# google/qhbm-library

Measured on AMD Instinct MI355X. Metric: circuit-expectation evals/sec (samples×Pauli terms) at n qubits; VQT step time, higher is better.
Workload: dtype f32; 1 GPU; BASELINE configs[2] (20-qubit XXZ, depth 16, 4096-sample VQT step): 20-qubit XXZ(delta=0.5) open chain, HEA depth 16 (944 params), 4096 states in total = 4096 on rank 0 of 1, VQT step = values + adjoint VJP; n_qubits=20, layers=16, states_total=4096, states_per_gpu=4096, pauli_terms=57, observables=1, hamiltonian=xxz, mode=vqt, parallelism=batch-sharded x1, backend_world_size=1, forward_passes=7, adjoint_passes=9

## Files before the change

### qhbm-library_amd/csrc/engine.cpp

```cpp
#include <hip/hip_runtime.h>

#include <algorithm>
#include <cmath>
#include <cstdio>
#include <iterator>
#include <cstdlib>
#include <cstring>
#include <memory>
#include <optional>
#include <string>
#include <vector>

#include "../../include/qhbm_engine.h"
#include "kernels.h"
#include "plan_args.h"
#include "program.h"
#include "schedule.h"

using namespace qhbm;

namespace {

std::string g_create_error;

// ... 46 lines not shown
  std::vector<std::pair<std::vector<char>, std::unique_ptr<DevicePlan>>> adj_cache;
  int64_t fwd_plans_built = 0, adj_plans_built = 0;
  DevBuf<DevTerm> global_terms;
  DevBuf<int> param_slot_begin, param_slots;
  DevBuf<float> slot_factor;
  DevBuf<ShiftPhase> shift_phases;
  int n_shift_phases = 0;
  bool shift_ready = false;
  size_t coef_batch_programs = 0;
};

struct TimedEvent {
  hipEvent_t a, b;
  int kind;
};

}

struct qhbm_engine {
  int device = -1;
  std::string err;
  Model model;
  bool have_circuit = false;
  int opt_tile = 0, opt_adj_tile = 0, opt_profile = 0, opt_round = 0;
  int opt_full_fwd = 60, opt_full_adj = 60, opt_force_general = 0;
  int opt_meas_tile = 0;
  int opt_values_from_obs = 1;
  bool retained_mu = false;
  int opt_cph_wave_bits = 1;
  int opt_fwd_values_obs = -1;
  int opt_adj_stop_early = -1;
  int opt_adj_plan_search = 1;
  int opt_wide_last = -1;
  int opt_fwd_pair = 1;
  int opt_shift_prefix = 1;
  int opt_adj_relabel = 1;
  int opt_obs_xcd_states = -1;
  int opt_x_two_shear = 1;
  int opt_adj_exchange = 1;
  int retained_U = 0;
  bool retained_table = false;
  int state_grad_U = 0;
  int64_t opt_chunk = 0;
  int64_t opt_budget_mb = 0;
  size_t resolved_budget = 0;
  bool plans_valid = false;
  bool adj_valid = false;
  std::vector<std::pair<std::vector<char>, std::unique_ptr<DevicePlan>>> adj_cache;
  int64_t fwd_plans_built = 0, adj_plans_built = 0;
  bool model_uploaded = false;
  DevicePlan fwd, adj;
  DevBuf<DevTerm> terms, global_terms;
  DevBuf<ObsGroup> obs_groups;
  bool terms_by_op = false;
  DevBuf<ObsBTerm> obs_bterms;
  DevBuf<ObsBGroup> obs_bgroups;
  uint32_t n_obs_bgroups = 0;
  int opt_obs_block_bits = kObsBlockBits;
  int opt_obs_split_rows = 0;
  int opt_obs_kernel = -1;
  mutable int block_choice = -1;
  int opt_gather_multi = 0;
  int opt_multi_values = -1;
  DevBuf<uint64_t> probe_out;
  DevBuf<float> probe_sink;
  DevBuf<float> value_part;
// ... 234 lines not shown
  }
  for (size_t i = 0; i < args->size(); ++i) {
    PassArgs& a = (*args)[i];
    if ((a.flags & PASS_INIT_BASIS) && (a.flags & PASS_NO_ZERO_FILL))
      for (uint32_t k = 0; k < a.n_nonlocal; ++k) a.zero_mask |= 1u << a.nonlocal_pos[k];
    a.n_free = a.n_nonlocal - uint32_t(__builtin_popcount(a.zero_mask));
  }
}

namespace {

double pass_flops_per_amplitude(const Plan& plan, const Pass& p, const uint32_t* dyn = nullptr);

double adjoint_plan_seconds(const Plan& plan, const Model& m) {
  std::vector<PassArgs> args;
  std::vector<uint32_t> prog, tables;
  fill_args(plan, m, &args, &prog, &tables);
  const double amps = double(size_t(1) << plan.n_eff);
  double t = 0.0;
  for (size_t i = 0; i < args.size(); ++i) {
    const Pass& p = plan.passes[i];
    const double live = 1.0 / double(1ull << __builtin_popcount(args[i].zero_mask));
    int low_missing = 0;
    for (uint32_t k = 0; k < args[i].n_nonlocal; ++k) low_missing += args[i].nonlocal_pos[k] < 4;
    const double lines = std::min(1.0, live * double(1u << low_missing));
    const double write_share = (p.flags & PASS_RELABEL) ? 1.0 / double(1u << __builtin_popcount(p.frozen_new_local)) : 1.0;
    const double bytes = lines * amps * 8.0 * 2.0 * (1.0 + ((p.flags & PASS_STORE) ? write_share : 0.0));
    const double flops = live * amps * pass_flops_per_amplitude(plan, p);
    t += std::max(flops / 67e12, bytes / 5.5e12) + 0.1 * bytes / 5.5e12;
  }
  return t;
}

int build_plans(qhbm_engine* h) {
  if (h->plans_valid && h->adj_valid) return 0;
  if (!h->have_circuit) return fail(h, "qhbm_set_circuit has not been called");
  if (h->model.n_ops > kMaxOps) return fail(h, "too many observables (max 1024)");
  std::string err;
  if (!h->plans_valid) {
    h->adj_cache.clear();
    if (!build_plan(h->model, h->opt_tile, h->opt_round, false, &h->fwd.plan, &err, h->opt_full_fwd, h->opt_meas_tile,
                    h->opt_cph_wave_bits != 0, false, h->opt_wide_last))
      return fail(h, "forward plan: " + err);
    h->fwd.uploaded = false;
    ++h->fwd_plans_built;
  }
  const bool relabel = h->opt_adj_relabel != 0 && h->opt_adj_exchange != 0;
  auto plan_adjoint_of = [&](const Model& model, int tile, Plan* out, double* seconds, std::string* e) {
    if (!build_plan(model, tile, 0, true, out, e, h->opt_full_adj, 0, h->opt_cph_wave_bits != 0, relabel)) return false;
    *seconds = adjoint_plan_seconds(*out, model);
    if (!h->opt_adj_plan_search) return true;
    const std::vector<std::vector<uint32_t>> orders = out->candidate_orders;
    for (const std::vector<uint32_t>& order : orders) {
      Plan alt;
      std::string e2;
      if (!build_plan(model, tile, 0, true, &alt, &e2, h->opt_full_adj, 0, h->opt_cph_wave_bits != 0, relabel, -1, &order))
        continue;
      const double f = adjoint_plan_seconds(alt, model);
      if (std::getenv("QHBM_PLAN_DEBUG"))
        std::fprintf(stderr, "[plan] tile %d candidate with %zu passes: %.4g ms per state (kept so far: %zu passes, %.4g ms)\n", tile,
                     alt.passes.size(), f * 1e3, out->passes.size(), *seconds * 1e3);
      if (f < 0.99 * *seconds) { *out = std::move(alt); *seconds = f; }
    }
    return true;
  };
  auto plan_adjoint = [&](int tile, Plan* out, double* seconds, std::string* e) {
    bool any_live = false;
    for (const Gate& G : h->model.gates) any_live |= G.param_idx >= 0 && !h->model.frozen(G.param_idx);
    if (h->opt_adj_stop_early == 0 && !h->model.param_frozen.empty() && any_live) {
      Model whole = h->model;
      whole.stop_at_first_live_gate = false;
      return plan_adjoint_of(whole, tile, out, seconds, e);
    }
    if (!plan_adjoint_of(h->model, tile, out, seconds, e)) return false;
    if (h->opt_adj_stop_early < 0 && !h->model.param_frozen.empty() && out->dense_tail) {
      Model whole = h->model;
// ... 958 lines not shown
    for (int j = term_offsets[k]; j < term_offsets[k + 1]; ++j) bound += std::fabs(double(coeffs[j]));
    int e = 0;
    if (bound > 0.0) (void)std::frexp(bound, &e);
    e = std::max(-60, std::min(60, e));
    h->h_op_scale[size_t(k)] = float(std::ldexp(1.0, kValueFracBits - e));
    h->h_op_inv_scale[size_t(k)] = float(std::ldexp(1.0, e - kValueFracBits));
  }
  h->model.n_ops = n_ops;
  h->model.terms = std::move(terms);
  invalidate_plans(h);
  h->block_choice = -1;
  h->terms.release();
  return 0;
}

int qhbm_set_option(qhbm_engine* h, const char* name, int64_t value) {
  if (!h || !name) return 1;
  const std::string k(name);
  if (k == "tile_qubits") { h->opt_tile = int(value); invalidate_plans(h); h->block_choice = -1; }
  else if (k == "round_qubits") { h->opt_round = int(value); invalidate_plans(h); }
  else if (k == "force_general_kernels") h->opt_force_general = int(value);
  else if (k == "full_diag_threshold") { h->opt_full_fwd = int(value); invalidate_plans(h); }
  else if (k == "adjoint_full_diag_threshold") { h->opt_full_adj = int(value); invalidate_plans(h); }
  else if (k == "adjoint_tile_qubits") { h->opt_adj_tile = int(value); invalidate_plans(h); }
  else if (k == "adjoint_exchange") { h->opt_adj_exchange = int(value); invalidate_plans(h); }
  else if (k == "x_two_shear") { h->opt_x_two_shear = value != 0; invalidate_plans(h); h->adj_cache.clear(); h->dense.adj_cache.clear(); }
  else if (k == "adjoint_relabel") { h->opt_adj_relabel = int(value); invalidate_plans(h); }
  else if (k == "forward_pairs") h->opt_fwd_pair = int(value);
  else if (k == "shift_prefix_sharing") { h->opt_shift_prefix = int(value); h->shift_ready = false; }
  else if (k == "forward_values_from_observable") h->opt_fwd_values_obs = int(value);
  else if (k == "adjoint_stop_early") { h->opt_adj_stop_early = int(value); invalidate_plans(h); }
  else if (k == "adjoint_plan_search") { h->opt_adj_plan_search = int(value); invalidate_plans(h); }
  else if (k == "wide_last_pass") { h->opt_wide_last = int(value); invalidate_plans(h); }
  else if (k == "observable_xcd_states") h->opt_obs_xcd_states = int(value);
  else if (k == "observable_kernel") { h->opt_obs_kernel = int(value); h->block_choice = -1; }
  else if (k == "observable_split_rows") h->opt_obs_split_rows = value != 0;
  else if (k == "observable_block_bits") {
    if (value != kObsBlockBits && value != kObsBlockBitsSmall) return fail(h, "observable_block_bits: 12 or 13");
    h->opt_obs_block_bits = int(value); h->block_choice = -1; h->terms.release(); h->model_uploaded = false;
  }
  else if (k == "multi_observable_values") h->opt_multi_values = int(value);
  else if (k == "gather_multi_values") h->opt_gather_multi = int(value);
  else if (k == "observable_far_windows") { h->opt_far_windows = int(value); h->terms.release(); h->model_uploaded = false; }
  else if (k == "measure_tile_qubits") { h->opt_meas_tile = int(value); invalidate_plans(h); }
  else if (k == "values_from_observable") h->opt_values_from_obs = int(value);
  else if (k == "cph_wave_bits") { h->opt_cph_wave_bits = int(value); invalidate_plans(h); }
  else if (k == "chunk_states") h->opt_chunk = value;
  else if (k == "evolve_step_argument") {
    if (value < 1 || value > 64) return fail(h, "evolve_step_argument: 1 .. 64");
    h->opt_evolve_step = int(value);
  }
  else if (k == "workspace_budget_mb") h->opt_budget_mb = std::max<int64_t>(0, value);
  else if (k == "profile_events") h->opt_profile = int(value);
  else return fail(h, "unknown option '" + k + "'");
  return 0;
}

int qhbm_workspace_bytes(qhbm_engine* h, int U, int with_vjp, size_t* out) {
  if (!h || !out) return 1;
  if (int rc = build_plans(h)) return rc;
  const uint32_t cs = with_vjp ? adjoint_chunk_states(h, U) : chunk_states(h, U);
  size_t b = size_t(cs) * state_bytes(h) * (with_vjp ? 2 : 1);
  if (with_vjp) {
    b += size_t(U) * h->adj.plan.slot_gate.size() * sizeof(float);
    size_t rows = 0;
    for (const Pass& p : h->adj.plan.passes)
// ... 1020 lines not shown
    HIPCHK(h->vals_tmp.reserve(nv));
    d_out_vals = h->vals_tmp.p;
  }
  std::vector<float> up(nv);
  for (int k = 0; k < T; ++k) {
    for (size_t i = 0; i < nv; ++i) up[i] = (int(i % size_t(T)) == k) ? 1.f : 0.f;
    HIPCHK(hipMemcpyAsync(h->upstream_tmp.p, up.data(), nv * sizeof(float), hipMemcpyHostToDevice, s));
    HIPCHK(hipStreamSynchronize(s));
    if (int rc = adjoint_sweep(h, d_bits, U, d_params, h->upstream_tmp.p, d_out_vals, s)) return rc;
    HIPCHK(launch_scatter_jac(h->state_grad.p, uint32_t(U), uint32_t(h->adj.plan.slot_gate.size()),
                              h->param_slot_begin.p, h->param_slots.p, h->slot_factor.p, d_jac, uint32_t(T),
                              uint32_t(k), uint32_t(P), s));
  }
  return 0;
}

int qhbm_num_passes(qhbm_engine* h, int* forward_passes, int* backward_passes) {
  if (!h) return 1;
  if (int rc = build_plans(h)) return rc;
  if (forward_passes) *forward_passes = int(h->fwd.plan.passes.size());
  if (backward_passes) *backward_passes = int(h->adj.plan.passes.size());
  return 0;
}

int qhbm_describe_schedule(qhbm_engine* h, char* buf, size_t buf_len) {
  if (!h || !buf || !buf_len) return 1;
  if (int rc = build_plans(h)) return rc;
  std::string s = describe_plan(h->fwd.plan) + describe_plan(h->adj.plan);
  {
    char line[96];
    std::snprintf(line, sizeof(line), "adjoint time model: %.2f us per state\n", 1e6 * adjoint_plan_seconds(h->adj.plan, h->model));
    s += line;
  }
  if (!h->model.terms.empty()) {
    s += std::string("observable kernel: lambda = ") + (block_kernel(h) ? "observable_blocks_kernel" : "apply_observable_kernel");
    s += std::string(" values = ") + (gather_multi_mode(h) ? "apply_observable_kernel (an accumulator per observable)"
                                      : multi_value_mode(h) || (value_mode(h) && block_kernel(h)) ? "observable_blocks_kernel"
                                      : value_mode(h)                                            ? "apply_observable_kernel"
                                                                                                  : "measured in the passes");
    s += "\n";
  }
  std::snprintf(buf, buf_len, "%s", s.c_str());
  return 0;
}

int qhbm_kernel_time_ms(qhbm_engine* h, int reset, double* fwd_ms, int64_t* fwd_launches, double* bwd_ms,
                        int64_t* bwd_launches, double* obs_ms, int64_t* obs_launches) {
  if (!h) return 1;
  double ms[3] = {0.0, 0.0, 0.0};
  int64_t cnt[3] = {0, 0, 0};
  if (h->device >= 0 && !h->events.empty()) {
    HIPCHK(hipSetDevice(h->device));
    HIPCHK(hipEventSynchronize(h->events.back().b));
    for (auto& ev : h->events) {
      float t = 0.f;
      if (hipEventElapsedTime(&t, ev.a, ev.b) == hipSuccess) { ms[ev.kind] += t; ++cnt[ev.kind]; }
    }
  }
  if (fwd_ms) *fwd_ms = ms[0];
  if (fwd_launches) *fwd_launches = cnt[0];
  if (bwd_ms) *bwd_ms = ms[1];
  if (bwd_launches) *bwd_launches = cnt[1];
  if (obs_ms) *obs_ms = ms[2];
  if (obs_launches) *obs_launches = cnt[2];
  if (reset) {
    h->free_events.insert(h->free_events.end(), h->events.begin(), h->events.end());
// ... 236 lines not shown
  if (with_vjp) {
    std::vector<PassArgs> args;
    std::vector<uint32_t> prog, tables;
    fill_args(h->adj.plan, h->model, &args, &prog, &tables);
    for (size_t i = 0; i < args.size(); ++i) {
      const double live = 1.0 / double(1ull << __builtin_popcount(args[i].zero_mask));
      b += live * amps * pass_flops_per_amplitude(h->adj.plan, h->adj.plan.passes[i], dyn_b.empty() ? nullptr : dyn_b.data());
    }
  }
  if (fwd_flops) *fwd_flops = f;
  if (obs_flops) *obs_flops = o;
  if (bwd_flops) *bwd_flops = b;
  return 0;
}

extern "C" {

int qhbm_traffic_model(qhbm_engine* h, int U, int with_vjp, double* fwd_bytes, double* obs_bytes,
                       double* bwd_bytes) {
  if (!h) return 1;
  if (int rc = build_plans(h)) return rc;
  const double tile_all = double(state_bytes(h)) * double(U);
  double f = 0.0, o = 0.0, b = 0.0;
  bool measure_only_after = !h->fwd.plan.global_terms.empty();
  for (const Pass& p : h->fwd.plan.passes) measure_only_after |= p.is_measure_only;
  const bool from_obs = with_vjp ? (value_mode(h) || multi_value_mode(h)) : forward_values_from_observable(h);
  {
    std::vector<PassArgs> fargs;
    std::vector<uint32_t> fprog, ftables;
    fill_args(h->fwd.plan, h->model, &fargs, &fprog, &ftables);
    for (size_t i = 0; i < fargs.size(); ++i) {
      const Pass& p = h->fwd.plan.passes[i];
      if (from_obs && p.is_measure_only) continue;
      const double live = 1.0 / double(1ull << __builtin_popcount(fargs[i].zero_mask));
      if (!(p.flags & PASS_INIT_BASIS)) f += live * tile_all;
      if (!p.is_measure_only && (!p.completes_circuit || from_obs || with_vjp || measure_only_after)) f += live * tile_all;
    }
  }
  if (!with_vjp && from_obs) o = tile_all;
  if (with_vjp) {
    o = 2.0 * tile_all;
    if (multi_value_mode(h) && !gather_multi_mode(h)) o += tile_all;
    std::vector<PassArgs> args;
    std::vector<uint32_t> prog, tables;
    fill_args(h->adj.plan, h->model, &args, &prog, &tables);
    for (size_t i = 0; i < args.size(); ++i) {
      double live = 1.0 / double(1ull << __builtin_popcount(args[i].zero_mask));
      {
        int low_missing = 0;
        for (uint32_t k = 0; k < args[i].n_nonlocal; ++k) low_missing += args[i].nonlocal_pos[k] < 4;
        live = std::min(1.0, live * double(1u << low_missing));
      }
      const Pass& ap = h->adj.plan.passes[i];
      double write_share = 1.0;
      if (ap.flags & PASS_RELABEL) write_share = 1.0 / double(1u << __builtin_popcount(ap.frozen_new_local));
      b += live * tile_all * 2.0 * (1.0 + ((ap.flags & PASS_STORE) ? write_share : 0.0));
    }
  }
  if (fwd_bytes) *fwd_bytes = f;
  if (obs_bytes) *obs_bytes = o;
  if (bwd_bytes) *bwd_bytes = b;
  return 0;
}

}
```

### qhbm-library_amd/csrc/kernels.hip

```cpp
#include <hip/hip_runtime.h>
#include <stdint.h>
#include <cstdio>
#include <cstring>

#include <utility>

#include "../../include/qhbm_engine.h"
#include "device_common.h"
#include "kernels.h"
#include "program.h"
#include "x_shear.h"

namespace qhbm {

namespace {


__device__ __forceinline__ uint32_t swz(uint32_t l) { return l ^ ((l >> 5) & 31u); }

constexpr int wg_per_cu(int lds_bytes) { return (160 * 1024) / lds_bytes < 1 ? 1 : (160 * 1024) / lds_bytes; }
constexpr int clampi(int v, int lo, int hi) { return v < lo ? lo : (v > hi ? hi : v); }
constexpr int fwd_lds(int K) { return (8 << K) + 8 * kMaxOps; }
constexpr int adj_lds(int K) { return (16 << K) + 4 * kMaxSlotsPerPass * ((1 << (K - 4)) / 64 < 1 ? 1 : (1 << (K - 4)) / 64); }
constexpr int adjx_lds(int K) { return (8 << K) + 4 * kMaxSlotsPerPass * ((1 << (K - 4)) / 64 < 1 ? 1 : (1 << (K - 4)) / 64); }
// ... 877 lines not shown
#pragma unroll
    for (int i = 0; i < NR; ++i)
      if (!(i >> s & 1)) {
        const float x = w[i], y = w[i | (1 << s)];
        w[i] = x + y;
        w[i | (1 << s)] = x - y;
      }
  wht_lane_stage<0>(w, lane);
  wht_lane_stage<1>(w, lane);
  wht_lane_stage<2>(w, lane);
  wht_lane_stage<3>(w, lane);
  wht_lane_stage<4>(w, lane);
  wht_lane_stage<5>(w, lane);
  uint32_t begin = 0;
#pragma unroll
  for (int c = 0; c < NR; ++c) {
    const uint32_t end = uni(class_end[c]);
    if (end != begin) {
      scr[lane] = w[c];
      for (uint32_t k = begin + uint32_t(lane); k < end; k += 64u) {
        const uint32_t* tw = terms + size_t(k) * kMeasTermWords;
        const uint4 t = make_uint4(tw[0], tw[1], tw[2], tw[3]);
        const uint32_t par = uint32_t(__popc(tile_base & t.y) + __popc(wave & (t.x >> 6))) & 1u;
        const float v = __uint_as_float(t.z ^ (par << 31)) * scr[t.x & 63u];
        atomicAdd(&red[t.w], to_fixed(v, op_scale[t.w]));
      }
    }
    begin = end;
  }
}

}

template <int K, int R, bool GEN>
__global__ __launch_bounds__(1 << (K - R), fwd_min_waves(K, R)) void pass_fwd_kernel(
    PassArgs a, float2* __restrict__ psi, const int8_t* __restrict__ bits, int n_user,
    const uint32_t* __restrict__ prog_base, const uint32_t* __restrict__ tables,
    const float* __restrict__ coef, const float* __restrict__ op_scale, unsigned long long* __restrict__ out64,
    uint32_t state0, const float2* __restrict__ psi_src) {
  constexpr int NT = 1 << (K - R);
  constexpr int NR = 1 << R;
  extern __shared__ __attribute__((aligned(16))) unsigned char smem[];
  float2* tile = reinterpret_cast<float2*>(smem);
  unsigned long long* red = reinterpret_cast<unsigned long long*>(tile + (1 << K));

  const int tid = threadIdx.x;
  const int lane = tid & 63;
  const uint32_t s_local = blockIdx.x >> a.n_free;
  uint32_t bits_row = state0 + s_local, out_row = state0 + s_local;
  if (a.prog_states) {
    const uint32_t q = s_local / a.prog_states;
    bits_row = state0 + (s_local - q * a.prog_states);
    out_row = s_local;
    coef += size_t(q) * a.coef_stride;
  }
  const uint32_t* recs = reinterpret_cast<const uint32_t*>(coef);
  TileCtx t = pass_tile_ctx(a, tables);
  const ThreadOff toff = thread_offsets(t, tid);
  uint32_t idx = 0;
  if ((a.flags & PASS_INIT_BASIS) | a.zero_mask | a.frozen_old_local) idx = input_index(a, bits + size_t(bits_row) * n_user, n_user, lane);
  const uint32_t in_local = local_bits<K>(a, idx, lane);
  const uint32_t tile_id = launched_tile(a, blockIdx.x, idx, lane);
  t.tile_base = tile_base_of(a, tile_id, lane);
  const uint32_t tile_hi = tile_id << K;
  float2* st = psi + (size_t(s_local) << a.n);

  if (a.flags & PASS_INIT_BASIS) {
    if ((idx & a.nonlocal_mask) != t.tile_base) {
      if ((a.flags & PASS_STORE) && !(a.flags & PASS_NO_ZERO_FILL)) {
        for (int p = tid; p < (1 << (K - 1)); p += NT)
          *reinterpret_cast<float4*>(st + global_index(t, 2u * p)) = make_float4(0.f, 0.f, 0.f, 0.f);
      }
      return;
    }
    for (int l = tid; l < (1 << K); l += NT) tile[l] = make_float2(0.f, 0.f);
    __syncthreads();
    if (tid == 0) tile[swz(in_local)] = make_float2(1.f, 0.f);
  } else {
    TileRegs r;
    const float2* ld = psi_src ? psi_src + (size_t(bits_row - state0) << a.n) : st;
    prefetch_tile<K, NT>(r, ld, t, toff);
    if (a.frozen_old_local) clear_stale<K>(r, tid, in_local, a.frozen_old_local);
    commit_tile<K, NT>(tile, r, tid);
  }
  for (int i = tid; i < kMaxOps; i += NT) red[i] = 0ull;
  __syncthreads();

  const uint32_t* prog = prog_base + a.prog_off;
  uint32_t pc = 0;
  constexpr int NV = 1;
  uint32_t cur[NV], nxt[NV];
  uint32_t carried_off = 0xffffffffu;
  for (;;) {
    const uint32_t w0 = uni(prog[pc]);
    const uint32_t opc = w0 & 0xffu;
    if (opc == OP_END) break;
    if (opc == OP_ROUND) {
      const uint32_t n_inst = (w0 & ~kRoundNoBarrier) >> 8;
      const uint32_t regmask = uni(prog[pc + 1]);
      uint32_t rec_off = uni(prog[pc + 2]);
      constexpr RecordLayout L(R, false);
      if (rec_off != carried_off) rec_load<NV>(recs, rec_off, lane, cur);
      uint32_t DB[R], T;
      const uint32_t TL = tables[a.tl_off + uni(prog[pc + 3]) + uint32_t(tid)];
      round_geometry<K, R>(regmask, TL, DB, &T);
      v2f amp[NR];
      round_load<R>(tile, T, DB, amp);
      for (uint32_t i = 0; i < n_inst; ++i) {
        rec_load<NV>(recs, rec_off + L.words(), lane, nxt);
        instance_fwd<R, NV, GEN>(cur, recs, rec_off, lane, amp, TL | tile_hi);
        rec_off += L.words();
#pragma unroll
        for (int v = 0; v < NV; ++v) cur[v] = nxt[v];
      }
// ... 55 lines not shown
              const float v = wave_sum(acc);
              if ((tid & 63) == 0) atomicAdd(&red[cur_op], to_fixed(v, op_scale[cur_op]));
            }
            acc = 0.f;
            cur_op = op;
          }
          float sfac = (ny == 1 || ny == 2) ? -cf : cf;
          if (__popc(t.tile_base & zn) & 1) sfac = -sfac;
          if (__popc(uint32_t(tid) & zl) & 1) sfac = -sfac;
          const uint32_t zhi = zl >> (K - R);
          const uint32_t key = zhi | ((ny & 1u) << 16);
          if (key != last_key) {
            sum = (ny & 1) ? meas_sum<R, 1>(w, zhi) : meas_sum<R, 0>(w, zhi);
            last_key = key;
          }
          acc = fmaf(sfac, sum, acc);
        }
      }
      if (cur_op != 0xffffffffu) {
        const float v = wave_sum(acc);
        if ((tid & 63) == 0) atomicAdd(&red[cur_op], to_fixed(v, op_scale[cur_op]));
      }
      __syncthreads();
    }
  }

  if (a.n_ops) {
    __syncthreads();
    for (uint32_t i = tid; i < a.n_ops; i += NT) {
      const unsigned long long v = red[i];
      if (v) atomicAdd(&out64[size_t(out_row) * a.n_ops + i], v);
    }
  }
  if (a.flags & PASS_STORE) store_tile<K, NT>(tile, st, t, thread_offsets(t, tid), tid);
}

template <int K>
__global__ __launch_bounds__(1 << (K - 4), adjx_min_waves(K)) void pass_fwd2_kernel(
    PassArgs a, float2* __restrict__ psi, const int8_t* __restrict__ bits, int n_user, uint32_t state0,
    const uint32_t* __restrict__ prog_base, const uint32_t* __restrict__ tables, const float* __restrict__ coef,
    uint32_t n_states) {
  constexpr int R = 4;
  constexpr int NT = 1 << (K - R);
  constexpr int NR = 1 << R;
  extern __shared__ __attribute__((aligned(16))) unsigned char smem[];
  float2* xt = reinterpret_cast<float2*>(smem);
  lds_tile_at_zero(smem);
  const int tid = threadIdx.x;
  const int lane = tid & 63;
  const uint32_t* recs = reinterpret_cast<const uint32_t*>(coef);
  const uint32_t tile_id = blockIdx.x & ((1u << a.n_nonlocal) - 1u);
  const uint32_t pair = blockIdx.x >> a.n_nonlocal;
  const uint32_t s_a = 2u * pair, s_b = min(2u * pair + 1u, n_states - 1u);
  TileCtx t = pass_tile_ctx(a, tables);
  const ThreadOff toff = thread_offsets(t, tid);
  t.tile_base = tile_base_of(a, tile_id, lane);
  const uint32_t tile_hi = tile_id << K;
  float2* st_a = psi + (size_t(s_a) << a.n);
  float2* st_b = psi + (size_t(s_b) << a.n);
  const uint32_t* prog = prog_base + a.prog_off;
  uint32_t w0 = uni(prog[0]);
  if ((w0 & 0xffu) != OP_ROUND) return;
  constexpr RecordLayout L(R, false);
  uint32_t pc = 0;
  uint32_t cur[1], nxt[1];
  uint32_t rec_off = uni(prog[2]);
  rec_load<1>(recs, rec_off, lane, cur);
// ... 1063 lines not shown
                                   uint32_t n_ops, uint32_t op, uint32_t n_params) {
  const uint32_t i = blockIdx.x * blockDim.x + threadIdx.x;
  if (i >= U * n_params) return;
  const uint32_t s = i / n_params, p = i % n_params;
  float acc = 0.f;
  for (int k = param_slot_begin[p]; k < param_slot_begin[p + 1]; ++k) {
    const int slot = param_slots[k];
    acc += slot_factor[slot] * state_grad[size_t(s) * n_slots + slot];
  }
  jac[(size_t(s) * n_ops + op) * n_params + p] = acc;
}

constexpr int kMaxDevices = 64;
size_t fwd_lds_bytes(int K) { return size_t(fwd_lds(K)); }
size_t adj_lds_bytes(int K, bool exchange) { return size_t(exchange ? adjx_lds(K) : adj_lds(K)); }

template <typename Kernel>
static hipError_t opt_in_lds(Kernel kernel, bool (&done)[kMaxDevices], size_t lds) {
  int dev = 0;
  if (hipError_t e = hipGetDevice(&dev); e != hipSuccess) return e;
  if (dev < 0 || dev >= kMaxDevices || !done[dev]) {
    hipError_t e = hipFuncSetAttribute(reinterpret_cast<const void*>(kernel),
                                       hipFuncAttributeMaxDynamicSharedMemorySize, int(lds));
    if (e != hipSuccess) return e;
    if (dev >= 0 && dev < kMaxDevices) done[dev] = true;
  }
  return hipSuccess;
}

static bool pass_prologue_ok(int K, const PassArgs& a, int n_user) {
  return K >= 10 && n_user >= 1 && n_user <= 32 && a.n >= 1u && a.n <= 32u && a.n_nonlocal <= 32u;
}

template <int K, int R, bool GEN>
static hipError_t launch_fwd_t(const PassArgs& a, uint32_t n_states, float2* psi, const int8_t* bits,
                               int n_user, const uint32_t* prog, const uint32_t* tables,
                               const float* coef, const float* op_scale, unsigned long long* out64, uint32_t state0,
                               hipStream_t stream, const float2* psi_src) {
  const size_t lds = fwd_lds_bytes(K);
  static bool attr_done[kMaxDevices] = {};
  if (hipError_t e = opt_in_lds(&pass_fwd_kernel<K, R, GEN>, attr_done, lds); e != hipSuccess) return e;
  const uint32_t grid = n_states << a.n_free;
  hipLaunchKernelGGL((pass_fwd_kernel<K, R, GEN>), dim3(grid), dim3(1 << (K - R)), lds, stream, a, psi, bits,
                     n_user, prog, tables, coef, op_scale, out64, state0, psi_src);
  return hipGetLastError();
}

hipError_t launch_pass_fwd(int K, int R, const PassArgs& a, uint32_t n_states, float2* psi, const int8_t* bits,
                           int n_user, const uint32_t* prog, const uint32_t* tables, const float* coef,
                           const float* op_scale, unsigned long long* out64, uint32_t state0, hipStream_t stream,
                           const float2* psi_src) {
  if (!pass_prologue_ok(K, a, n_user)) return hipErrorInvalidValue;
  if (psi_src && ((a.flags & PASS_INIT_BASIS) || !a.prog_states)) return hipErrorInvalidValue;
#define QHBM_FWD_CASE(K_, R_)                                                                          \
  if (K == K_ && R == R_)                                                                              \
    return (a.flags & PASS_GENERAL)                                                                    \
               ? launch_fwd_t<K_, R_, true>(a, n_states, psi, bits, n_user, prog, tables, coef, op_scale, out64, state0, stream, psi_src)   \
               : launch_fwd_t<K_, R_, false>(a, n_states, psi, bits, n_user, prog, tables, coef, op_scale, out64, state0, stream, psi_src);
  QHBM_FWD_CASE(10, 4)
  QHBM_FWD_CASE(11, 4)
  QHBM_FWD_CASE(12, 4)
  QHBM_FWD_CASE(13, 4)
  QHBM_FWD_CASE(14, 4)
#undef QHBM_FWD_CASE
  return hipErrorInvalidValue;
}

template <int K>
static hipError_t launch_fwd2_t(const PassArgs& a, uint32_t n_states, float2* psi, const int8_t* bits, int n_user,
                                uint32_t state0, const uint32_t* prog, const uint32_t* tables, const float* coef,
                                hipStream_t stream) {
  const size_t lds = size_t(8) << K;
  static bool attr_done[kMaxDevices] = {};
  if (hipError_t e = opt_in_lds(&pass_fwd2_kernel<K>, attr_done, lds); e != hipSuccess) return e;
  const uint32_t grid = ((n_states + 1u) / 2u) << a.n_nonlocal;
  hipLaunchKernelGGL((pass_fwd2_kernel<K>), dim3(grid), dim3(1 << (K - 4)), lds, stream, a, psi, bits, n_user, state0, prog,
                     tables, coef, n_states);
  return hipGetLastError();
}

bool pass_fwd_pair_supported(int K) { return K >= 10 && K <= 13; }

hipError_t launch_pass_fwd_pair(int K, const PassArgs& a, uint32_t n_states, float2* psi, const int8_t* bits, int n_user,
                                uint32_t state0, const uint32_t* prog, const uint32_t* tables, const float* coef,
                                hipStream_t stream) {
  if (!pass_prologue_ok(K, a, n_user)) return hipErrorInvalidValue;
  switch (K) {
// ... 837 lines not shown
```

### qhbm-library_amd/csrc/schedule.cpp

```cpp
#include "schedule.h"

#include <algorithm>
#include <cmath>
#include <cstdio>
#include <cstdlib>
#include <cstring>
#include <sstream>

#include "../../include/qhbm_engine.h"

namespace qhbm {
namespace {

inline int popc(uint32_t x) { return __builtin_popcount(x); }

bool odd_constant(const Gate& G) {
  if (G.param_idx >= 0) return false;
  const float t = G.offset;
  return t == std::nearbyint(t) && (long(std::nearbyint(t)) & 1L);
}

bool lower(const Model& m, std::vector<LoweredOp>* ops, std::string* err, double* const_phase = nullptr,
           std::vector<std::pair<int, float>>* phases = nullptr) {
  ops->clear();
// ... 693 lines not shown
      ++p->n_meas_groups;
    }
    if (which.empty()) return;
    p->prog.push_back(OP_MEASURE | (uint32_t(which.size()) << 8));
    for (int gi : which) {
      const MeasGroup& g = groups[gi];
      p->prog.push_back(to_local(*p, g.x));
      p->prog.push_back(uint32_t(g.terms.size()));
      for (int ti : g.terms) {
        const PauliTerm& t = m_.terms[ti];
        uint32_t cb;
        std::memcpy(&cb, &t.coeff, 4);
        p->prog.push_back(to_local(*p, t.z & S));
        p->prog.push_back(t.z & ~S);
        p->prog.push_back(cb);
        p->prog.push_back(uint32_t(t.op) | (uint32_t(t.ny & 3) << 24));
        ++p->n_meas_terms;
      }
      ++p->n_meas_groups;
    }
  }

 private:
  const Model& m_;
  int K_, R_, n_eff_;
  bool adjoint_;
  Plan* plan_;
};

}

bool build_plan(const Model& m, int tile_bits, int round_bits, bool adjoint, Plan* plan, std::string* err,
                int full_threshold, int meas_tile_bits, bool cph_wave_bits, bool relabel, int wide_last_pass,
                const std::vector<uint32_t>* forced_order) {
  *plan = Plan();
  plan->full_threshold = full_threshold;
  plan->cph_wave_bits = cph_wave_bits;
  plan->tail_tiles = cph_wave_bits;
  if (m.n < 1 || m.n > kMaxQubits - 1) { *err = "n_qubits must be in [1, 31]"; return false; }
  const int n_eff = std::max(m.n, kMinTileBits);
  const int k_cap = adjoint ? kMaxTileBits - 1 : kMaxTileBits;
  int K;
  if (tile_bits == 0) {
    K = n_eff <= k_cap ? n_eff : (adjoint || n_eff <= 21 ? 12 : 13);
  } else {
    if (tile_bits < kMinTileBits || tile_bits > k_cap) {
      *err = "tile_qubits out of range";
      return false;
    }
    K = std::min(n_eff, tile_bits);
  }
  const int R = kRoundBits;
  if (round_bits != 0 && round_bits != kRoundBits) {
    *err = "round_qubits must be 4";
    return false;
  }
  plan->n = m.n;
  plan->n_eff = n_eff;
  plan->K = K;
  plan->R = R;
  plan->adjoint = adjoint;
  plan->dense_input = m.dense_input;

  std::vector<LoweredOp> ops;
  if (!lower(m, &ops, err, &plan->const_phase, &plan->gate_phases)) return false;
  uint32_t always_pending = 0;
  if (adjoint && !m.param_frozen.empty() && m.stop_at_first_live_gate) {
// ... 252 lines not shown
    }
  }
  if (!planned.empty() && !forced_order) {
    std::vector<char> dn(done);
    std::vector<int> gphys(phys);
    uint32_t gfrozen = frozen;
    size_t left = ops.size() - n_done, greedy_passes = 0;
    std::vector<uint32_t> greedy_sets;
    while (left) {
      int best_mat = -1;
      size_t best_total = 0;
      uint32_t best_set = 0;
      std::vector<int> best;
      for (uint32_t S : gen_cands(dn, gphys)) {
        int n_mat = 0;
        std::vector<int> lst = absorb_capped(dn, S, &n_mat);
        if (n_mat > best_mat || (n_mat == best_mat && lst.size() > best_total)) { best_mat = n_mat; best_total = lst.size(); best_set = S; best.swap(lst); }
      }
      if (best.empty()) break;
      for (int oi : best) dn[size_t(oi)] = 1;
      left -= best.size();
      ++greedy_passes;
      greedy_sets.push_back(best_set);
      if (plan->relabel && left) relabel_after(best_set, dn, &gphys, &gfrozen);
    }
    std::sort(complete.begin(), complete.end(), [](const auto& x, const auto& y) { return x.first < y.first; });
    for (const auto& c : complete) {
      if (plan->candidate_orders.size() >= 6) break;
      if (c.second != planned) plan->candidate_orders.push_back(c.second);
    }
    if (left == 0) plan->candidate_orders.push_back(greedy_sets);
    if (left == 0 && planned.size() > greedy_passes + (plan->relabel ? 4 : 1)) planned.clear();
  }
  size_t planned_i = 0;
  {
    if (const char* env = std::getenv(adjoint ? "QHBM_ADJ_SETS" : "QHBM_FWD_SETS")) {
      planned.clear();
      for (const char* q = env; *q;) {
        char* end = nullptr;
        const unsigned long v = std::strtoul(q, &end, 16);
        if (end == q) break;
        planned.push_back(uint32_t(v));
        q = *end ? end + 1 : end;
      }
    }
  }

  while (n_done < ops.size()) {
    std::vector<uint32_t> cands = planned_i < planned.size() ? std::vector<uint32_t>{planned[planned_i++]} : gen_cands(done, phys);
    int wide_K = 0;
    uint32_t wide_S = 0;
    const bool widen = wide_last_pass > 0 || (wide_last_pass < 0 && tile_bits == 0);
    if (!adjoint && K < n_eff && plan->tail_tiles && widen && !plan->passes.empty() && !std::getenv("QHBM_NO_WIDE_LAST_PASS")) {
      uint32_t S = (1u << c_min) - 1;
      for (int oi : order) {
        if (done[oi]) continue;
        const LoweredOp& op = ops[oi];
        S |= op.type == LOW_DIAG ? (op.bits & S ? 0u : (op.bits & (0u - op.bits))) : op.bits;
      }
      const int need = popc(S);
      if (need > K && need <= std::min(K + 2, std::min(n_eff, 13))) {
        wide_K = need;
        wide_S = S;
      }
    }
    if (!adjoint && K < n_eff && !groups.empty()) {
      uint32_t S = (1u << c_min) - 1;
      bool fits = true;
      for (int oi : order) {
        if (done[oi]) continue;
        const LoweredOp& op = ops[oi];
        const uint32_t need = op.type == LOW_DIAG ? (op.bits & S ? 0u : (op.bits & (0u - op.bits))) : op.bits;
        if (popc(S | need) > K) { fits = false; break; }
        S |= need;
      }
      if (fits) {
        const int here = int(plan->passes.size());
        for (size_t gi = 0; gi < groups.size() && fits; ++gi) {
          const int ready = group_ready(gi, here);
          bool earlier = false;
          for (int pi = ready; pi < here && !earlier; ++pi) earlier = (groups[gi].x & ~pass_set(plan->passes[size_t(pi)])) == 0;
          if (earlier) continue;
          if (popc(S | groups[gi].x) <= K) S |= groups[gi].x; else fits = false;
        }
      }
      if (fits) {
        for (int bit = n_eff - 1; bit >= 0 && popc(S) < K; --bit) if (!(S >> bit & 1)) S |= 1u << bit;
        cands.insert(cands.begin(), S);
      }
    }
    uint32_t best_S = 0;
    int best_mat = -1;
    size_t best_total = 0;
    std::vector<int> best_list;
    std::vector<uint32_t> blocks;
    if (K < n_eff) {
      const uint32_t low = (1u << c_min) - 1;
      const int h = K - c_min;
      for (int pp = c_min; pp + h <= n_eff; ++pp) blocks.push_back(low | (((1u << h) - 1) << pp));
    }
    for (uint32_t S : cands) {
      int n_mat = 0;
      std::vector<int> lst = absorb_capped(done, S, &n_mat);
      int next_best = 0;
      if (!adjoint && !blocks.empty() && n_done + lst.size() < ops.size()) {
        std::vector<char> done2(done);
        for (int oi : lst) done2[oi] = 1;
        for (uint32_t S2 : blocks) {
          int m2 = 0;
          absorb(ops, order, done2, S2, all_bits, &m2);
          next_best = std::max(next_best, m2);
        }
      }
      const int score = n_mat + next_best;
      if (score > best_mat || (score == best_mat && lst.size() > best_total)) {
        best_mat = score; best_total = lst.size(); best_S = S; best_list.swap(lst);
      }
    }
    if (best_list.empty()) { *err = "scheduler made no progress"; return false; }
    Builder wide(m, wide_K ? wide_K : K, R, n_eff, adjoint, plan);
    Builder* bp = &b;
    if (wide_K) {
      int n_mat = 0;
      std::vector<int> all_left = absorb(ops, order, done, wide_S, all_bits, &n_mat);
      if (all_left.size() == ops.size() - n_done) {
        best_S = wide_S;
        best_list.swap(all_left);
        bp = &wide;
      }
    }
    Pass p = bp->begin_pass(best_S, &phys);
    p.frozen_old_local = Builder::to_local(p, frozen & best_S);
    p.slot_base = int(plan->slot_gate.size());
    {
      std::vector<char> here(ops.size(), 0);
      for (int oi : best_list) here[size_t(oi)] = 1;
      uint32_t pend = always_pending;
      for (size_t oi = 0; oi < ops.size(); ++oi)
        if (!done[oi] && !here[oi] && ops[oi].type != LOW_DIAG) pend |= ops[oi].bits;
      bp->pending_mat_outside_ = pend;
    }
    if (!bp->emit_ops(&p, ops, best_list, err)) return false;
    {
      uint32_t mixed = 0;
      for (int oi : best_list) if (ops[size_t(oi)].type != LOW_DIAG) mixed |= ops[size_t(oi)].bits;
      static_assert(LOW_MAT2 == 3, "a new LoweredType must be classified here: diagonal, or reported in mat_bits");
      if (mixed != p.mat_bits) { *err = "internal: a non-diagonal op of the pass is missing from mat_bits"; return false; }
    }
    for (int oi : best_list) { done[oi] = 1; op_pass[oi] = int(plan->passes.size()); ++n_done; }
    if (plan->relabel && n_done < ops.size()) {
      const std::vector<int> before(phys);
      const uint32_t f_new = relabel_after(best_S, done, &phys, &frozen);
// ... 180 lines not shown
        }
      os << "; by group (X+PH1 | PH2 | CPH | Y+dense) low-half only / high-half only / both:";
      for (int g8 = 0; g8 < 4; ++g8) os << " " << half[g8][0] << "/" << half[g8][1] << "/" << half[g8][2];
      os << "\n";
      int at[4][8] = {}, sets[16] = {};
      for (uint32_t off : p.record_offsets) {
        int m = 0;
        for (int g8 = 0; g8 < 4; ++g8)
          for (int v = 0; v < 8; ++v)
            if (p.coef_init[off + L.slot_lane8(g8, v)] != 0xffffffffu) { ++at[g8][v]; m |= 1 << g8; }
        ++sets[m];
      }
      os << "  slots at value position 0..7, by group:";
      for (int g8 = 0; g8 < 4; ++g8)
        for (int v = 0; v < 8; ++v) os << (v ? "/" : " ") << at[g8][v];
      os << "; records by sets reduced 0..15:";
      for (int m = 0; m < 16; ++m) os << (m ? "/" : " ") << sets[m];
      os << "\n";
    }
    os << "  census: instances=" << n_inst << " (FULL " << n_full << ") X=" << x << " PH1=" << ph1 << " PH2=" << ph2
       << " FULL-PH1=" << fph1 << " FULL-PH2=" << fph2 << " CPH=" << cph << " (tile predicate " << cph_tile << ") slot-groups=" << groups << " instances by X count 0..4: " << x_hist[0] << "/" << x_hist[1] << "/"
       << x_hist[2] << "/" << x_hist[3] << "/" << x_hist[4] << " X-in-FULL=" << x_full << "\n";
  }
  for (size_t i = 0; i < p.passes.size(); ++i) {
    const Pass& q = p.passes[i];
    os << "  pass " << i << ": K=" << q.K << " c=" << q.c << " local=[";
    for (size_t k = 0; k < q.local_pos.size(); ++k) os << (k ? "," : "") << q.local_pos[k];
    os << "] mat_ops=" << q.n_mat_ops << " diag_terms=" << q.n_diag_terms << " rounds=" << q.n_rounds
       << " instances=" << q.n_instances << " meas_groups=" << q.n_meas_groups
       << " meas_terms=" << q.n_meas_terms << " slots=" << q.n_slots
       << (q.is_measure_only ? " [measure-only]" : "");
    if (!p.adjoint && (q.flags & PASS_INIT_BASIS)) os << ((q.flags & PASS_NO_ZERO_FILL) ? " [basis tile only]" : " [zero-fill]");
    if (!p.adjoint && p.dense_input && i == 0) os << " [loads caller states]";
    os << " words=" << q.prog.size() << " regs=";
    for (size_t r = 0; r < q.round_regmasks.size(); ++r) os << (r ? "," : "") << std::hex << q.round_regmasks[r] << std::dec;
    if (p.relabel) {
      os << " at=";
      for (size_t k = 0; k < q.local_phys.size(); ++k) os << (k ? "," : "") << q.local_phys[k];
      if (q.flags & PASS_RELABEL) os << " moves-local-bits=" << std::hex << q.frozen_new_local << std::dec;
      if (q.frozen_old_local) os << " stale-local-bits=" << std::hex << q.frozen_old_local << std::dec;
    }
    {
      const RecordLayout L(p.R, p.adjoint);
      os << " x_full=";
      for (size_t r = 0; r < q.round_words.size(); ++r) {
        const uint32_t w0 = q.prog[q.round_words[r]], n_inst = (w0 & ~kRoundNoBarrier) >> 8, first = q.prog[q.round_words[r] + 2];
        int x = 0, xf = 0;
        for (uint32_t i = 0; i < n_inst; ++i) {
          const uint32_t* rec = &p.coef_init[first + size_t(i) * size_t(L.words())];
          x += __builtin_popcount(rec[0] & 0xfu);
          if (rec[1] & kFullDiagFlag) xf += __builtin_popcount(rec[0] & 0xfu);
        }
        os << (r ? "," : "") << xf << "/" << x;
      }
    }
    if (p.adjoint) {
      const RecordLayout L(p.R, true);
      size_t l1 = 0;
      for (size_t r = 0; r < q.round_words.size(); ++r) {
        const uint32_t w0 = q.prog[q.round_words[r]], n_inst = (w0 & ~kRoundNoBarrier) >> 8, first = q.prog[q.round_words[r] + 2];
        for (uint32_t i = 0; i < n_inst; ++i) l1 += size_t(level1_adds(&p.coef_init[first + size_t(i) * size_t(L.words())]));
      }
      os << " level1_adds=" << l1;
      os << " dead=";
      for (size_t r = 0; r < q.round_words.size(); ++r) os << (r ? "," : "") << std::hex << q.prog[q.round_words[r] + 4] << std::dec;
    }
// ... 76 lines not shown
```

### qhbm-library_amd/csrc/schedule.h

```cpp
#pragma once
#include <cstdint>
#include <string>
#include <vector>

#include "program.h"

namespace qhbm {

struct Gate {
  int32_t kind, q0, q1, param_idx;
  float scalar, offset;
  float global_shift;
};

struct PauliTerm {
  float coeff;
  uint32_t x, z;
  int ny;
  int op;
};

struct LoweredOp {
  int type = LOW_SKIP;
  int kind = 0;
// ... 31 lines not shown
  uint32_t frozen_new_local = 0;
  uint32_t frozen_old_local = 0;
  std::vector<uint32_t> relabel_tab;
  std::vector<uint32_t> prog;
  std::vector<uint32_t> spread;
  std::vector<uint32_t> round_tl;
  bool is_measure_only = false;
  bool completes_circuit = false;
  int n_mat_ops = 0, n_diag_terms = 0, n_rounds = 0, n_instances = 0;
  std::vector<uint32_t> round_regmasks;
  std::vector<uint32_t> round_wavemasks;
  std::vector<uint32_t> round_words;
  int n_meas_groups = 0, n_meas_terms = 0;
  int slot_base = 0, n_slots = 0;
  uint32_t mat_bits = 0;
};

struct Plan {
  int n = 0, n_eff = 0, K = 0, R = 0;
  bool adjoint = false;
  std::vector<Pass> passes;
  std::vector<CoefJob> jobs;
  int n_coef_floats = 0;
  std::vector<uint32_t> coef_init;
  std::vector<uint32_t> record_offsets;
  int full_threshold = 60;
  bool tail_tiles = true;
  bool relabel = false;
  bool cph_wave_bits = true;
  std::vector<int> global_terms;
  std::vector<int> slot_gate;
  std::vector<float> slot_factor;
  std::vector<std::vector<uint32_t>> candidate_orders;
  bool dense_tail = false;
  bool dense_input = false;
  double const_phase = 0.0;
  std::vector<std::pair<int, float>> gate_phases;
};

struct Model {
  int n = 0;
  int n_params = 0;
  std::vector<Gate> gates;
  std::vector<char> param_frozen;
  bool stop_at_first_live_gate = true;
  bool frozen(int param_idx) const { return param_idx >= 0 && size_t(param_idx) < param_frozen.size() && param_frozen[size_t(param_idx)]; }
  int n_ops = 0;
  std::vector<PauliTerm> terms;
  bool dense_input = false;
};


bool build_plan(const Model& m, int tile_bits, int round_bits, bool adjoint, Plan* out,
                std::string* err, int full_threshold = 60, int meas_tile_bits = 0, bool cph_wave_bits = true,
                bool relabel = false, int wide_last_pass = -1, const std::vector<uint32_t>* forced_order = nullptr);

std::string describe_plan(const Plan& p);

std::vector<int> first_dependent_pass(const Plan& plan, size_t n_gates, int* first_measuring);

struct ProgramOrder {
  std::vector<int> dst;
  std::vector<uint32_t> group_end;
  bool shares = false;
};
ProgramOrder order_programs(const Plan& fwd, size_t n_gates, const int* shift_gates, size_t n_programs, bool may_share,
                            bool values_outside_passes);

}
```

Before: 730,300 evals/s.

## Add cost-priced forward pass-order search and 8-row tile kernels for c=0 passes

Adds a forward-plan search. It derives candidate pass orders from a reverse (adjoint-style) schedule of the circuit, prices each with a roofline-style time model, and keeps the cheapest. The search sits behind a new `forward_search` option that is off by default. Separately, forward passes with c == 0 now launch specialised kernels built on ROWS8 thread offsets, so K=10..13 tiles are loaded and stored with fewer rows per thread. Traffic accounting now counts cache lines touched when low qubit bits are nonlocal. The new kernel routing rejects zero-filling init-basis store passes when c == 0 and fails any c == 0 shape outside K 10..13 with R=4, which could break plans that previously ran.

```diff
diff --git a/qhbm-library_amd/csrc/engine.cpp b/qhbm-library_amd/csrc/engine.cpp
--- a/qhbm-library_amd/csrc/engine.cpp
+++ b/qhbm-library_amd/csrc/engine.cpp
@@ -102,6 +102,9 @@
   int opt_adj_stop_early = -1;
   int opt_adj_plan_search = 1;
   int opt_wide_last = -1;
+  int opt_fwd_search = 0;
+  double fwd_seconds = 0.0, fwd_seconds_greedy = 0.0;
+  size_t fwd_orders_priced = 0;
   int opt_fwd_pair = 1;
   int opt_shift_prefix = 1;
   int opt_adj_relabel = 1;
@@ -402,6 +405,31 @@
   return t;
 }
 
+constexpr double kFwdFlops = 92e12, kFwdBytes = 4.5e12, kFwdSingle = 0.88;
+double forward_plan_seconds(const Plan& plan, const Model& m) {
+  std::vector<PassArgs> args;
+  std::vector<uint32_t> prog, tables;
+  fill_args(plan, m, &args, &prog, &tables);
+  const double amps = double(size_t(1) << plan.n_eff);
+  double t = 0.0;
+  for (size_t i = 0; i < args.size(); ++i) {
+    const Pass& p = plan.passes[i];
+    const double live = 1.0 / double(1ull << __builtin_popcount(args[i].zero_mask));
+    int low_missing = 0;
+    for (uint32_t k = 0; k < args[i].n_nonlocal; ++k) low_missing += args[i].nonlocal_pos[k] < 4;
+    const double lines = std::min(1.0, live * double(1u << low_missing));
+    const bool loads = !(p.flags & PASS_INIT_BASIS), stores = !p.is_measure_only;
+    const double bytes = lines * amps * 8.0 * ((loads ? 1.0 : 0.0) + (stores ? 1.0 : 0.0));
+    const bool pair = loads && !(p.flags & PASS_GENERAL) && args[i].zero_mask == 0 && !p.is_measure_only && p.K >= 10 && p.K <= 13;
+    const double flops = live * amps * pass_flops_per_amplitude(plan, p);
+    t += std::max(flops / (kFwdFlops * (pair ? 1.0 : kFwdSingle)), bytes / kFwdBytes) + 0.1 * bytes / kFwdBytes;
+    if (std::getenv("QHBM_PLAN_DEBUG"))
+      std::fprintf(stderr, "[plan]   forward pass %zu: live 2^-%d lines %.4f %s %.3f Mflop %.3f MB\n", i, __builtin_popcount(args[i].zero_mask),
+                   lines, pair ? "pair" : "single", flops * 1e-6, bytes * 1e-6);
+  }
+  return t;
+}
+
 int build_plans(qhbm_engine* h) {
   if (h->plans_valid && h->adj_valid) return 0;
   if (!h->have_circuit) return fail(h, "qhbm_set_circuit has not been called");
@@ -410,8 +438,30 @@
   if (!h->plans_valid) {
     h->adj_cache.clear();
     if (!build_plan(h->model, h->opt_tile, h->opt_round, false, &h->fwd.plan, &err, h->opt_full_fwd, h->opt_meas_tile,
-                    h->opt_cph_wave_bits != 0, false, h->opt_wide_last))
+                    h->opt_cph_wave_bits != 0, false, h->opt_wide_last, nullptr, h->opt_fwd_search != 0))
       return fail(h, "forward plan: " + err);
+    h->fwd_seconds_greedy = h->fwd_seconds = forward_plan_seconds(h->fwd.plan, h->model);
+    bool took = false;
+    const std::vector<std::vector<uint32_t>> orders = h->fwd.plan.candidate_orders;
+    h->fwd_orders_priced = 0;
+    const std::vector<std::vector<int>> stages = h->fwd.plan.candidate_stages;
+    for (size_t ci = 0; ci < orders.size() && ci < stages.size(); ++ci) {
+      Plan alt;
+      std::string e2;
+      ++h->fwd_orders_priced;
+      if (!build_plan(h->model, h->opt_tile, h->opt_round, false, &alt, &e2, h->opt_full_fwd, h->opt_meas_tile,
+                      h->opt_cph_wave_bits != 0, false, h->opt_wide_last, &orders[ci], false, &stages[ci]))
+        continue;
+      const double f = forward_plan_seconds(alt, h->model);
+      if (std::getenv("QHBM_PLAN_DEBUG"))
+        std::fprintf(stderr, "[plan] forward candidate with %zu passes: %.4g ms per state (kept so far: %zu passes, %.4g ms)\n",
+                     alt.passes.size(), f * 1e3, h->fwd.plan.passes.size(), h->fwd_seconds * 1e3);
+      if (f < 0.99 * h->fwd_seconds || (h->opt_fwd_search == 2 && (!took || f < h->fwd_seconds))) {
+        h->fwd.plan = std::move(alt);
+        h->fwd_seconds = f;
+        took = true;
+      }
+    }
     h->fwd.uploaded = false;
     ++h->fwd_plans_built;
   }
@@ -1436,6 +1486,7 @@
   else if (k == "adjoint_stop_early") { h->opt_adj_stop_early = int(value); invalidate_plans(h); }
   else if (k == "adjoint_plan_search") { h->opt_adj_plan_search = int(value); invalidate_plans(h); }
   else if (k == "wide_last_pass") { h->opt_wide_last = int(value); invalidate_plans(h); }
+  else if (k == "forward_search") { h->opt_fwd_search = int(value); invalidate_plans(h); }
   else if (k == "observable_xcd_states") h->opt_obs_xcd_states = int(value);
   else if (k == "observable_kernel") { h->opt_obs_kernel = int(value); h->block_choice = -1; }
   else if (k == "observable_split_rows") h->opt_obs_split_rows = value != 0;
@@ -2522,6 +2573,12 @@
     std::snprintf(line, sizeof(line), "adjoint time model: %.2f us per state\n", 1e6 * adjoint_plan_seconds(h->adj.plan, h->model));
     s += line;
   }
+  if (h->opt_fwd_search) {
+    char line[160];
+    std::snprintf(line, sizeof(line), "forward time model: %.2f us per state (greedy order: %.2f us; %zu searched orders priced)\n",
+                  1e6 * h->fwd_seconds, 1e6 * h->fwd_seconds_greedy, h->fwd_orders_priced);
+    s += line;
+  }
   if (!h->model.terms.empty()) {
     s += std::string("observable kernel: lambda = ") + (block_kernel(h) ? "observable_blocks_kernel" : "apply_observable_kernel");
     s += std::string(" values = ") + (gather_multi_mode(h) ? "apply_observable_kernel (an accumulator per observable)"
@@ -2824,7 +2881,12 @@
     for (size_t i = 0; i < fargs.size(); ++i) {
       const Pass& p = h->fwd.plan.passes[i];
       if (from_obs && p.is_measure_only) continue;
-      const double live = 1.0 / double(1ull << __builtin_popcount(fargs[i].zero_mask));
+      double live = 1.0 / double(1ull << __builtin_popcount(fargs[i].zero_mask));
+      if (!(p.flags & PASS_INIT_BASIS)) {
+        int low_missing = 0;
+        for (uint32_t k = 0; k < fargs[i].n_nonlocal; ++k) low_missing += fargs[i].nonlocal_pos[k] < 4;
+        live = std::min(1.0, live * double(1u << low_missing));
+      }
       if (!(p.flags & PASS_INIT_BASIS)) f += live * tile_all;
       if (!p.is_measure_only && (!p.completes_circuit || from_obs || with_vjp || measure_only_after)) f += live * tile_all;
     }
diff --git a/qhbm-library_amd/csrc/kernels.hip b/qhbm-library_amd/csrc/kernels.hip
--- a/qhbm-library_amd/csrc/kernels.hip
+++ b/qhbm-library_amd/csrc/kernels.hip
@@ -933,7 +933,7 @@
 
 }
 
-template <int K, int R, bool GEN>
+template <int K, int R, bool GEN, int ROWS = ROWS16>
 __global__ __launch_bounds__(1 << (K - R), fwd_min_waves(K, R)) void pass_fwd_kernel(
     PassArgs a, float2* __restrict__ psi, const int8_t* __restrict__ bits, int n_user,
     const uint32_t* __restrict__ prog_base, const uint32_t* __restrict__ tables,
@@ -957,7 +957,7 @@
   }
   const uint32_t* recs = reinterpret_cast<const uint32_t*>(coef);
   TileCtx t = pass_tile_ctx(a, tables);
-  const ThreadOff toff = thread_offsets(t, tid);
+  const ThreadOff toff = thread_offsets<ROWS>(t, tid);
   uint32_t idx = 0;
   if ((a.flags & PASS_INIT_BASIS) | a.zero_mask | a.frozen_old_local) idx = input_index(a, bits + size_t(bits_row) * n_user, n_user, lane);
   const uint32_t in_local = local_bits<K>(a, idx, lane);
@@ -980,7 +980,7 @@
   } else {
     TileRegs r;
     const float2* ld = psi_src ? psi_src + (size_t(bits_row - state0) << a.n) : st;
-    prefetch_tile<K, NT>(r, ld, t, toff);
+    prefetch_tile<K, NT, ROWS>(r, ld, t, toff);
     if (a.frozen_old_local) clear_stale<K>(r, tid, in_local, a.frozen_old_local);
     commit_tile<K, NT>(tile, r, tid);
   }
@@ -1102,7 +1102,7 @@
       if (v) atomicAdd(&out64[size_t(out_row) * a.n_ops + i], v);
     }
   }
-  if (a.flags & PASS_STORE) store_tile<K, NT>(tile, st, t, thread_offsets(t, tid), tid);
+  if (a.flags & PASS_STORE) store_tile<K, NT, ROWS>(tile, st, t, thread_offsets<ROWS>(t, tid), tid);
 }
 
 template <int K>
@@ -2232,16 +2232,16 @@
   return K >= 10 && n_user >= 1 && n_user <= 32 && a.n >= 1u && a.n <= 32u && a.n_nonlocal <= 32u;
 }
 
-template <int K, int R, bool GEN>
+template <int K, int R, bool GEN, int ROWS = ROWS16>
 static hipError_t launch_fwd_t(const PassArgs& a, uint32_t n_states, float2* psi, const int8_t* bits,
                                int n_user, const uint32_t* prog, const uint32_t* tables,
                                const float* coef, const float* op_scale, unsigned long long* out64, uint32_t state0,
                                hipStream_t stream, const float2* psi_src) {
   const size_t lds = fwd_lds_bytes(K);
   static bool attr_done[kMaxDevices] = {};
-  if (hipError_t e = opt_in_lds(&pass_fwd_kernel<K, R, GEN>, attr_done, lds); e != hipSuccess) return e;
+  if (hipError_t e = opt_in_lds(&pass_fwd_kernel<K, R, GEN, ROWS>, attr_done, lds); e != hipSuccess) return e;
   const uint32_t grid = n_states << a.n_free;
-  hipLaunchKernelGGL((pass_fwd_kernel<K, R, GEN>), dim3(grid), dim3(1 << (K - R)), lds, stream, a, psi, bits,
+  hipLaunchKernelGGL((pass_fwd_kernel<K, R, GEN, ROWS>), dim3(grid), dim3(1 << (K - R)), lds, stream, a, psi, bits,
                      n_user, prog, tables, coef, op_scale, out64, state0, psi_src);
   return hipGetLastError();
 }
@@ -2252,7 +2252,21 @@
                            const float2* psi_src) {
   if (!pass_prologue_ok(K, a, n_user)) return hipErrorInvalidValue;
   if (psi_src && ((a.flags & PASS_INIT_BASIS) || !a.prog_states)) return hipErrorInvalidValue;
-#define QHBM_FWD_CASE(K_, R_)                                                                          \
+  if (a.c == 0) {
+    if ((a.flags & PASS_INIT_BASIS) && (a.flags & PASS_STORE) && !(a.flags & PASS_NO_ZERO_FILL)) return hipErrorInvalidValue;
+#define QHBM_FWD_CASE8(K_)                                                                                                                         \
+  if (K == K_ && R == 4)                                                                                                                           \
+    return (a.flags & PASS_GENERAL)                                                                                                                \
+               ? launch_fwd_t<K_, 4, true, ROWS8>(a, n_states, psi, bits, n_user, prog, tables, coef, op_scale, out64, state0, stream, psi_src)    \
+               : launch_fwd_t<K_, 4, false, ROWS8>(a, n_states, psi, bits, n_user, prog, tables, coef, op_scale, out64, state0, stream, psi_src);
+    QHBM_FWD_CASE8(10)
+    QHBM_FWD_CASE8(11)
+    QHBM_FWD_CASE8(12)
+    QHBM_FWD_CASE8(13)
+#undef QHBM_FWD_CASE8
+    return hipErrorInvalidValue;
+  }
+#define QHBM_FWD_CASE(K_, R_)                                                                        \
   if (K == K_ && R == R_)                                                                              \
     return (a.flags & PASS_GENERAL)                                                                    \
                ? launch_fwd_t<K_, R_, true>(a, n_states, psi, bits, n_user, prog, tables, coef, op_scale, out64, state0, stream, psi_src)   \
diff --git a/qhbm-library_amd/csrc/schedule.cpp b/qhbm-library_amd/csrc/schedule.cpp
--- a/qhbm-library_amd/csrc/schedule.cpp
+++ b/qhbm-library_amd/csrc/schedule.cpp
@@ -749,7 +749,7 @@
 
 bool build_plan(const Model& m, int tile_bits, int round_bits, bool adjoint, Plan* plan, std::string* err,
                 int full_threshold, int meas_tile_bits, bool cph_wave_bits, bool relabel, int wide_last_pass,
-                const std::vector<uint32_t>* forced_order) {
+                const std::vector<uint32_t>* forced_order, bool forward_search, const std::vector<int>* forced_stage) {
   *plan = Plan();
   plan->full_threshold = full_threshold;
   plan->cph_wave_bits = cph_wave_bits;
@@ -1068,6 +1068,39 @@
     if (left == 0) plan->candidate_orders.push_back(greedy_sets);
     if (left == 0 && planned.size() > greedy_passes + (plan->relabel ? 4 : 1)) planned.clear();
   }
+  if (!adjoint && forward_search && !forced_order && K < n_eff && K <= kMaxTileBits - 1 && plan->tail_tiles &&
+      !m.dense_input && ever_mat == all_bits) {
+    Model rev = m;
+    rev.param_frozen.clear();
+    rev.terms.clear();
+    rev.n_ops = 0;
+    Plan back;
+    std::string ignored;
+    if (build_plan(rev, K, round_bits, true, &back, &ignored, full_threshold, 0, cph_wave_bits, false)) {
+      std::vector<int> backward(ops.size());
+      for (size_t i = 0; i < ops.size(); ++i) backward[i] = int(ops.size() - 1 - i);
+      auto offer = [&](const std::vector<uint32_t>& sets) {
+        std::vector<char> dn(ops.size(), 0);
+        std::vector<int> stage(ops.size(), 0);
+        size_t left = ops.size();
+        const int n_sets = int(sets.size());
+        for (int j = 0; j < n_sets && left; ++j) {
+          int n_mat = 0;
+          for (int oi : absorb(ops, backward, dn, sets[size_t(j)], all_bits, &n_mat)) { dn[size_t(oi)] = 1; stage[size_t(oi)] = n_sets - 1 - j; --left; }
+        }
+        if (left) return;
+        std::vector<uint32_t> fwd(sets.rbegin(), sets.rend());
+        if (std::find(plan->candidate_orders.begin(), plan->candidate_orders.end(), fwd) != plan->candidate_orders.end()) return;
+        plan->candidate_orders.push_back(std::move(fwd));
+        plan->candidate_stages.push_back(std::move(stage));
+      };
+      std::vector<uint32_t> chosen;
+      for (const Pass& q : back.passes) chosen.push_back(pass_set(q));
+      offer(chosen);
+      for (const std::vector<uint32_t>& o : back.candidate_orders) offer(o);
+    }
+  }
+  if (forced_stage && forced_stage->size() != ops.size()) { *err = "forced pass order: one stage per lowered op"; return false; }
   size_t planned_i = 0;
   {
     if (const char* env = std::getenv(adjoint ? "QHBM_ADJ_SETS" : "QHBM_FWD_SETS")) {
@@ -1083,7 +1116,11 @@
   }
 
   while (n_done < ops.size()) {
-    std::vector<uint32_t> cands = planned_i < planned.size() ? std::vector<uint32_t>{planned[planned_i++]} : gen_cands(done, phys);
+    bool from_order = planned_i < planned.size();
+    std::vector<int> staged;
+    if (from_order && forced_stage && !adjoint)
+      for (int oi : order) if ((*forced_stage)[size_t(oi)] <= int(planned_i)) staged.push_back(oi);
+    std::vector<uint32_t> cands = from_order ? std::vector<uint32_t>{planned[planned_i++]} : gen_cands(done, phys);
     int wide_K = 0;
     uint32_t wide_S = 0;
     const bool widen = wide_last_pass > 0 || (wide_last_pass < 0 && tile_bits == 0);
@@ -1121,6 +1158,12 @@
         }
       }
       if (fits) {
+        if (from_order && forced_stage) {
+          from_order = false;
+          planned_i = planned.size();
+          staged.clear();
+          cands = gen_cands(done, phys);
+        }
         for (int bit = n_eff - 1; bit >= 0 && popc(S) < K; --bit) if (!(S >> bit & 1)) S |= 1u << bit;
         cands.insert(cands.begin(), S);
       }
@@ -1137,7 +1180,7 @@
     }
     for (uint32_t S : cands) {
       int n_mat = 0;
-      std::vector<int> lst = absorb_capped(done, S, &n_mat);
+      std::vector<int> lst = from_order && forced_stage && !adjoint ? absorb(ops, staged, done, S, all_bits, &n_mat) : absorb_capped(done, S, &n_mat);
       int next_best = 0;
       if (!adjoint && !blocks.empty() && n_done + lst.size() < ops.size()) {
         std::vector<char> done2(done);
@@ -1153,7 +1196,9 @@
         best_mat = score; best_total = lst.size(); best_S = S; best_list.swap(lst);
       }
     }
+    if (best_list.empty() && from_order && !adjoint && forced_order) continue;
     if (best_list.empty()) { *err = "scheduler made no progress"; return false; }
+    if (from_order && forced_order && (popc(best_S) != K || (best_S & ~all_bits))) { *err = "forced pass order: a local set is not a tile"; return false; }
     Builder wide(m, wide_K ? wide_K : K, R, n_eff, adjoint, plan);
     Builder* bp = &b;
     if (wide_K) {
@@ -1400,6 +1445,11 @@
        << (q.is_measure_only ? " [measure-only]" : "");
     if (!p.adjoint && (q.flags & PASS_INIT_BASIS)) os << ((q.flags & PASS_NO_ZERO_FILL) ? " [basis tile only]" : " [zero-fill]");
     if (!p.adjoint && p.dense_input && i == 0) os << " [loads caller states]";
+    if (!p.adjoint && !q.is_measure_only) {
+      uint32_t low_out = 0;
+      for (int b : q.nonlocal_pos) if (b < std::min(p.K, 4)) low_out |= 1u << b;
+      if (low_out) os << " [head: low-bits-out=" << std::hex << low_out << std::dec << " rows=" << (q.c == 0 ? 8 : 16) << "]";
+    }
     os << " words=" << q.prog.size() << " regs=";
     for (size_t r = 0; r < q.round_regmasks.size(); ++r) os << (r ? "," : "") << std::hex << q.round_regmasks[r] << std::dec;
     if (p.relabel) {
diff --git a/qhbm-library_amd/csrc/schedule.h b/qhbm-library_amd/csrc/schedule.h
--- a/qhbm-library_amd/csrc/schedule.h
+++ b/qhbm-library_amd/csrc/schedule.h
@@ -87,6 +87,7 @@
   std::vector<int> slot_gate;
   std::vector<float> slot_factor;
   std::vector<std::vector<uint32_t>> candidate_orders;
+  std::vector<std::vector<int>> candidate_stages;
   bool dense_tail = false;
   bool dense_input = false;
   double const_phase = 0.0;
@@ -108,7 +109,8 @@
 
 bool build_plan(const Model& m, int tile_bits, int round_bits, bool adjoint, Plan* out,
                 std::string* err, int full_threshold = 60, int meas_tile_bits = 0, bool cph_wave_bits = true,
-                bool relabel = false, int wide_last_pass = -1, const std::vector<uint32_t>* forced_order = nullptr);
+                bool relabel = false, int wide_last_pass = -1, const std::vector<uint32_t>* forced_order = nullptr,
+                bool forward_search = false, const std::vector<int>* forced_stage = nullptr);
 
 std::string describe_plan(const Plan& p);
 
```

Result: no change. 731,000 evals/s, median of 2 (+0.1%).
